# DeepLearningZ/chanamq

Hardware: AMD Instinct MI355X
Metric: msgs/sec (whole node) + p50 publish→deliver latency, 1 KB payload, 1/2/4/8 GPUs (higher is better)
Workload: dtype uint8 (AMQP wire bytes; no floating-point compute)

## Files before the change

### csrc/kernels/dataplane.hip

```cpp
#include "dp_state.h"
#include "dp_util.h"

DEV void apply_deltas(const DS& d, const u8* buf, u32 tid, u32 nt, DeltaRec* lrec) {
  const DeltaHead h = *(const DeltaHead*)buf;
  const DeltaRec* recs = (const DeltaRec*)(buf + sizeof(DeltaHead));
  const u32* dirty = (const u32*)(recs + h.nrec);
  const uint4* data = (const uint4*)((const u8*)dirty + ((4u * h.ndirty + 15u) & ~15u));
  for (u32 r = tid; r < h.nrec; r += nt) lrec[r] = recs[r];
  __syncthreads();
  for (u32 i = tid; i < h.nchunk; i += nt) {
    u32 lo = 0, hi = h.nrec;
    while (hi - lo > 1) {
      const u32 mid = (lo + hi) >> 1;
      if (lrec[mid].chunk0 <= i) lo = mid; else hi = mid;
    }
    const DeltaRec r = lrec[lo];
    const u32 off = (i - r.chunk0) * 16u;
    const u32 n = r.len - off < 16u ? r.len - off : 16u;
    const uint4 v = data[i];
    u8* dst = (u8*)(uintptr_t)(r.dst + off);
    const u32 w[4] = {v.x, v.y, v.z, v.w};
    if (((uintptr_t)dst & 3) == 0 && (n & 3) == 0) {
      for (u32 k = 0; k < n / 4; ++k) ((u32*)dst)[k] = w[k];
    } else {
// ... 77 lines not shown
    const u32 o = block_scan<1024>(v, lds, all);
    if (k < nseg) { d.seg_total[k] = cl + len; d.seg_start[k] = run + o; }
    run += all;
  }
}

#include "dp_frame_scan.h"

DEV void set_counts(const DS& d, u32 np, u32 na) {
  d.ctr->n_pubs = np < d.pub_max ? np : d.pub_max;
  d.ctr->n_acks = na < d.ack_max ? na : d.ack_max;
  d.tot[TS_RANGE_LO] = 0;
  d.tot[TS_RANGE_HI] = d.ctr->n_pubs;
  d.tot[TS_PAIR_BASE] = 0;
  d.tot[TS_PAIR_N] = 0;
  d.tot[TS_NIMPORT] = 0;
}

DEV bool skip_shortstr(const u8* p, u32& o, u32 end) {
  if (o + 1 > end) return false;
  o += 1 + p[o];
  return o <= end;
}

DEV u32 build_keyvec(const DS& d, const u8* key, u32 len, u32 pi) {
  Words kw = words_of(key, len);
  if (d.tb_max) {
    uint4* kv = (uint4*)(d.pub_keyvec + (u64)pi * TOPIC_K);
    u16* kwo = d.pub_kwoff + (u64)pi * TOPIC_WORDS;
    u32 off = 0;
    u32 wi = 0;
    if (kw.count) {
      while (wi < TOPIC_WORDS && off <= kw.eff) {
        u32 wl = word_len(key, off, kw.eff);
        u32 h = fnv1a32(key + off, wl);
        kwo[wi] = (u16)((off << 8) | (wl & 255));
        u32 pk[8];
#pragma unroll
        for (int g = 0; g < 8; ++g) {
          u32 v = 0;
#pragma unroll
          for (int bb = 0; bb < 4; ++bb) v |= (((h >> (g * 4 + bb)) & 1) ? 0x01u : 0xffu) << (8 * bb);
          pk[g] = v;
        }
        kv[wi * 2] = make_uint4(pk[0], pk[1], pk[2], pk[3]);
        kv[wi * 2 + 1] = make_uint4(pk[4], pk[5], pk[6], pk[7]);
        off += wl + 1;
        ++wi;
      }
    }
    for (; wi < TOPIC_WORDS; ++wi) {
      kv[wi * 2] = make_uint4(0, 0, 0, 0);
      kv[wi * 2 + 1] = make_uint4(0, 0, 0, 0);
    }
  }
  return kw.count;
}

struct Win32 { u32 w0, w1, w2, w3, w4, w5, w6, w7; };
DEV Win32 load_win(const u8* p) {
  const U4 a = *(const U4*)p, b = *(const U4*)(p + 16);
  return Win32{a.x, a.y, a.z, a.w, b.x, b.y, b.z, b.w};
}
DEV u32 win_word(const Win32& s, u32 k) {
  const u32 a0 = s.w0, a1 = s.w1, a2 = s.w2, a3 = s.w3, a4 = s.w4, a5 = s.w5, a6 = s.w6, a7 = s.w7;
  const u32 lo = k < 2 ? (k == 0 ? a0 : a1) : (k == 2 ? a2 : a3);
  const u32 hi = k < 6 ? (k == 4 ? a4 : a5) : (k == 6 ? a6 : a7);
  return k < 4 ? lo : hi;
}
DEV u32 win_byte(const Win32& s, u32 i) { return (win_word(s, i >> 2) >> (8 * (i & 3))) & 255u; }
DEV u32 win_get(const Win32& s, u32 i) { return win_byte(s, i); }
template <u32 S>
DEV u64 win_fnv64(const Win32& s, u32 n, u64 h) {
#pragma unroll
  for (u32 i = 0; i + S < 32; ++i) {
    if (i < n) {
      h ^= win_byte(s, i + S);
      h *= FNV64_PRIME;
    }
  }
  return h;
}

DEV u32 build_keyvec_win(const DS& d, const Win32& s, u32 n, u32 pi) {
  const u32 lenmask = n >= 32 ? ~0u : ((1u << n) - 1u);
  u32 dots = 0;
#pragma unroll
  for (u32 i = 0; i < 32; ++i) dots |= (win_byte(s, i) == '.' ? 1u : 0u) << i;
  dots &= lenmask;
  const u32 nd = ~dots & lenmask;
  const u32 eff = nd ? 32u - __clz(nd) : 0u;
  const u32 effmask = eff >= 32 ? ~0u : ((1u << eff) - 1u);
  const u32 de = dots & effmask;
  const u32 count = n == 0 ? 1u : (eff == 0 ? 0u : 1u + __popc(de));
  if (!d.tb_max) return count;
  u32 hw[TOPIC_WORDS];
#pragma unroll
  for (u32 k = 0; k < TOPIC_WORDS; ++k) hw[k] = 0x811c9dc5u;
  u32 h = 0x811c9dc5u, wi = 0;
#pragma unroll
  for (u32 i = 0; i < 32; ++i) {
    const u32 c = win_byte(s, i);
    const bool in = i < eff, dot = in && c == '.';
#pragma unroll
    for (u32 k = 0; k < TOPIC_WORDS; ++k) hw[k] = (dot && wi == k) ? h : hw[k];
    wi += dot ? 1u : 0u;
    h = dot ? 0x811c9dc5u : (in ? (h ^ c) * 0x01000193u : h);
  }
#pragma unroll
  for (u32 k = 0; k < TOPIC_WORDS; ++k) hw[k] = wi == k ? h : hw[k];
  const u32 nw = count < TOPIC_WORDS ? count : TOPIC_WORDS;
  uint4* kv = (uint4*)(d.pub_keyvec + (u64)pi * TOPIC_K);
  u16* kwo = d.pub_kwoff + (u64)pi * TOPIC_WORDS;
  u32 off = 0;
#pragma unroll
  for (u32 k = 0; k < TOPIC_WORDS; ++k) {
    if (k < nw) {
      const u32 rest = off >= 32 ? 0u : (de & ~((1u << off) - 1u));
      u32 e = rest ? (u32)(__ffs(rest) - 1) : eff;
      if (e > eff) e = eff;
      const u32 wl = e - off;
      kwo[k] = (u16)((off << 8) | (wl & 255));
      u32 pk[8];
#pragma unroll
      for (int g = 0; g < 8; ++g) {
        u32 v = 0;
#pragma unroll
        for (int bb = 0; bb < 4; ++bb) v |= (((hw[k] >> (g * 4 + bb)) & 1) ? 0x01u : 0xffu) << (8 * bb);
        pk[g] = v;
      }
      kv[k * 2] = make_uint4(pk[0], pk[1], pk[2], pk[3]);
      kv[k * 2 + 1] = make_uint4(pk[4], pk[5], pk[6], pk[7]);
      off = e + 1;
    } else {
      kv[k * 2] = make_uint4(0, 0, 0, 0);
      kv[k * 2 + 1] = make_uint4(0, 0, 0, 0);
    }
  }
  return count;
}

DEV void apply_ack(const DS& d, Ack a, u32 ai) {
  const u32 ch = a.chslot;
  if (ch == INVALID) { d.acks[ai] = a; return; }
  const u64 nt = d.ch_next_tag[ch];
  u64 tag = a.tag;
  if (tag == 0 && a.multiple) tag = nt - 1;
  a.tag = tag;
  d.acks[ai] = a;
  const bool requeue = (a.kind != CK_ACK) && a.requeue;
  if (a.multiple) {
    atomicMin(&d.ch_mlo[ch], ai);
    atomicMax(&d.ch_mhi[ch], ai);
  } else if (tag >= d.ch_uhead[ch] && tag < nt) {
    USlot& u = d.uwin[(u64)ch * (d.ucap_mask + 1) + ((tag - 1) & d.ucap_mask)];
    atomicCAS(&u.state, (u32)US_PENDING, requeue ? (u32)US_REQUEUE : (u32)US_ACKED);
  }
  if (atomicExch(&d.ch_dirty[ch], 1u) == 0) {
    u32 k = atomicAdd(d.n_dirty, 1u);
    d.dirty_list[k] = ch;
  }
  atomicAdd(&d.ctr->n_acked, 1u);
}

__global__ __launch_bounds__(256) void k_decode(DS d) {
  __shared__ u32 spref[DEC_SEG_LDS];
  __shared__ u32 sprefa[DEC_SEG_LDS];
  __shared__ u32 lds[256 / 64 + 1];
  const u32 nseg = d.in->nseg;
  const bool seg_order = nseg <= DEC_SEG_LDS;
  u32 n0 = d.ctr->n_cmds;
  n0 = n0 < d.cmd_max ? n0 : d.cmd_max;
  if (!d.rank_scan) {
    if (blockIdx.x != 0 && blockIdx.x * 256 >= n0) return;
    u32 run = 0, runa = 0;
    for (u32 b0 = 0; b0 < nseg; b0 += 256) {
      const u32 k = b0 + threadIdx.x;
      const u32 v = k < nseg ? d.seg_npub[k] : 0, va = k < nseg ? d.seg_nack[k] : 0;
      u32 all, alla;
      const u32 o = block_scan<256>(v, lds, all);
      const u32 oa = block_scan<256>(va, lds, alla);
      if (k < nseg) { spref[k] = run + o; sprefa[k] = runa + oa; }
      run += all;
      runa += alla;
    }
    if (blockIdx.x == 0 && threadIdx.x == 0) set_counts(d, run, runa);
    __syncthreads();
    if (blockIdx.x * 256 >= n0) return;
  } else {
    if (blockIdx.x == 0 && threadIdx.x == 0) set_counts(d, d.tot[TS_CMD_PUBS], d.tot[TS_CMD_ACKS]);
    if (blockIdx.x * 256 >= n0) return;
    if (seg_order) {
      u32 run = 0;
      for (u32 b0 = 0; b0 < nseg; b0 += 256) {
        const u32 k = b0 + threadIdx.x;
        const u32 v = k < nseg ? d.seg_npub[k] : 0;
        u32 all;
        const u32 o = block_scan<256>(v, lds, all);
        if (k < nseg) spref[k] = run + o;
        run += all;
      }
      __syncthreads();
    }
  }
  u32 i = blockIdx.x * blockDim.x + threadIdx.x;
  u32 n = d.ctr->n_cmds;
  if (n > d.cmd_max) n = d.cmd_max;
  if (i >= n) return;
  const Cmd c = d.cmds[i];
  const u8* w = d.work;
  if (c.kind == CK_PUBLISH) {
    u32 pi;
    if (!d.rank_scan) {
      pi = spref[c.seg] + c.pad[1];
    } else {
      pi = d.cmd_pub_rank[i];
      if (seg_order && c.seg < nseg && d.seg_cmd_base[c.seg] != INVALID)
        pi = spref[c.seg] + (pi - d.cmd_pub_rank[d.seg_cmd_base[c.seg]]);
    }
    if (pi >= d.pub_max) return;
    Pub pb;
    pb.conn = c.conn;
    pb.chslot = c.pad[0];
    pb.frag0 = c.frag0;
    pb.nfrag = c.nfrag;
    pb.body_size = c.body_size;
    pb.flags = 0;
    pb.expire_ms = 0;
    pb.ts_ms = 0;
    pb.nq = 0; pb.slot_bytes = 0; pb.msg = INVALID; pb.pad = 0; pb.xid = 0;
    u32 o = c.m_off + 6, end = c.m_off + c.m_len;
    const u32 o0 = o;
    const Win32 ma = load_win(w + o0);
    bool ok = o <= end;
    pb.ex_off = o + 1;
    const u32 b0 = ok && o < end ? win_byte(ma, 0) : 0u;
    pb.ex_len = b0;
    if (ok) { if (o + 1 > end) ok = false; else { o += 1 + b0; ok = o <= end; } }
    pb.rk_off = o + 1;
    const u32 b1 = ok && o < end ? (o - o0 < 32 ? win_get(ma, o - o0) : (u32)w[o]) : 0u;
    pb.rk_len = b1;
    if (ok) { if (o + 1 > end) ok = false; else { o += 1 + b1; ok = o <= end; } }
    const Win32 rkw = load_win(w + pb.rk_off);
    u32 bits = (ok && o < end) ? (o - pb.rk_off < 32 ? win_get(rkw, o - pb.rk_off) : (u32)w[o]) : 0u;
    if (bits & 1) pb.flags |= MF_MANDATORY;
    if (bits & 2) pb.flags |= MF_IMMEDIATE;
    i32 xs = -1;
    if (ok) {
      const u32 vh = d.conn_vhost[c.conn];
      u64 hk = pb.ex_len <= 31 ? win_fnv64<1>(ma, pb.ex_len, FNV64_BASIS ^ (u64(vh) * 0x9E3779B97F4A7C15ULL))
                               : exch_hash(vh, w + pb.ex_off, pb.ex_len);
      u32 mask = d.xhash_mask;
      for (u32 j = 0; j <= mask; ++j) {
        u32 slot = (u32)(hk + j) & mask;
        i32 v = d.x_hval[slot];
        if (v < 0) break;
        if (d.x_hkey[slot] == hk) { xs = v; break; }
      }
    }
    pb.exch = ok ? xs : -2;
    pb.keyhash = pb.rk_len <= 32 ? win_fnv64<0>(rkw, pb.rk_len, FNV64_BASIS) : fnv1a64_dev(w + pb.rk_off, pb.rk_len);
    u32 ho = c.h_off + 12, hend = c.h_off + c.h_len;
    pb.props_off = ho;
    pb.props_len = hend > ho ? hend - ho : 0;
    const Win32 pw = load_win(w + ho);
    auto pbyte = [&](u32 q) -> u32 { const u32 o = q - ho; return o < 32 ? win_byte(pw, o) : (u32)w[q]; };
    u32 fl = 0;
    u32 nfl = 0;
    u32 q = ho;
    while (q + 2 <= hend) {
      u32 fw = (pbyte(q) << 8) | pbyte(q + 1);
      q += 2;
      if (nfl == 0) fl = fw;
      ++nfl;
      if (!(fw & 1)) break;
    }
    bool pok = true;
    for (int bit = 15; bit >= 2 && pok; --bit) {
      if (!(fl & (1u << bit))) continue;
      switch (bit) {
        case 13: {
          if (q + 4 > hend) { pok = false; break; }
          u32 tl = (pbyte(q) << 24) | (pbyte(q + 1) << 16) | (pbyte(q + 2) << 8) | pbyte(q + 3);
          q += 4 + tl;
          pok = q <= hend;
          break;
        }
        case 12:
          if (q + 1 > hend) { pok = false; break; }
          if (pbyte(q) == 2) pb.flags |= MF_PERSIST;
          q += 1;
          break;
        case 11: q += 1; pok = q <= hend; break;
        case 8: {
          if (q + 1 > hend) { pok = false; break; }
          u32 sl = pbyte(q);
          if (q + 1 + sl > hend) { pok = false; break; }
          i64 v = 0;
          bool digits = sl > 0 && sl <= 18;
          for (u32 k = 0; k < sl && digits; ++k) {
            u32 ch = pbyte(q + 1 + k);
            if (ch < '0' || ch > '9') digits = false;
            else v = v * 10 + (ch - '0');
          }
          if (digits) pb.expire_ms = d.in->now_ms + v;
          q += 1 + sl;
          break;
        }
        case 6: {
          if (q + 8 > hend) { pok = false; break; }
          u64 ts = 0;
#pragma unroll
          for (u32 k = 0; k < 8; ++k) ts = (ts << 8) | pbyte(q + k);
          pb.ts_ms = (i64)ts * 1000;
          pb.flags |= MF_HAS_TS;
          q += 8;
          break;
        }
        default:
          if (q + 1 > hend) { pok = false; break; }
          q += 1 + pbyte(q);
          pok = q <= hend;
      }
    }
    pb.nwords = pb.rk_len <= 32 ? build_keyvec_win(d, rkw, pb.rk_len, pi) : build_keyvec(d, w + pb.rk_off, pb.rk_len, pi);
    if (c.nfrag == 1 && d.in->ingress_host && d.in->ref_back != 0xffffffffu && c.body_size >= d.in->ref_min &&
        c.seg < nseg) {
      const Frag fg = d.frags[c.frag0];
      const u32 w0 = d.seg_start[c.seg], cl = d.seg_total[c.seg] - d.segs[c.seg].len;
      const u64 ing_rel = (u64)d.in->ingress - (u64)d.work;
      if (fg.len == c.body_size && d.scan_inplace && (u64)d.in->ingress > (u64)d.work && fg.off >= ing_rel) {
        pb.flags |= MF_HREF;
        pb.pad = (u32)(fg.off - ing_rel);
      } else if (fg.len == c.body_size && fg.off >= w0 + cl && fg.off < w0 + d.seg_total[c.seg]) {
        pb.flags |= MF_HREF;
        pb.pad = (u32)(d.segs[c.seg].src + (fg.off - w0 - cl));
      }
    }
    d.pubs[pi] = pb;
  } else if (c.kind == CK_ACK || c.kind == CK_NACK || c.kind == CK_REJECT) {
    const u32 ai = d.rank_scan ? d.cmd_ack_rank[i] : sprefa[c.seg] + c.pad[2];
    if (ai >= d.ack_max) return;
    Ack a;
    a.chslot = c.pad[0];
    a.kind = c.kind;
    u32 o = c.m_off + 4;
    bool ok = c.m_len >= 13;
    a.tag = ok ? be64(w + o) : 0;
    u32 bits = ok ? w[o + 8] : 0;
    if (c.kind == CK_ACK) { a.multiple = bits & 1; a.requeue = 0; }
    else if (c.kind == CK_REJECT) { a.multiple = 0; a.requeue = bits & 1; }
    else { a.multiple = bits & 1; a.requeue = (bits >> 1) & 1; }
    d.acks[ai] = a;
  }
}

DEV void marks_range(const DS& d, u32 i0, u32 stride) {
  if (i0 == 0 && d.links)
    for (u32 r = 0; r < WORLD_MAX; ++r) d.lk_cnt[r] = 0;
  const u32 na = d.ctr->n_acks, np = d.ctr->n_pubs;
  const u32 n = na > np ? na : np;
  for (u32 i = i0; i < n; i += stride) {
    if (i < na) apply_ack(d, d.acks[i], i);
    if (i < np) {
      const u32 ch = d.pubs[i].chslot;
      if (ch != INVALID && d.ch_confirm[ch]) atomicAdd(&d.ch_pub_cnt[ch], 1u);
    }
  }
}

struct ScanArgs { const u32* in[4]; u32* out[4]; const u32* n; const u32* lo; u32 narr; u32 nmax; u32 tot_slot; u64 stride; };
#define SCAN_TILE 4096
template <int NA, int EPT>
DEV bool scan_tile(const ScanArgs& a, u32* tot, u64* status, u32* ctl, u32 smax) {
  constexpr u32 TILE = 1024 * EPT;
  __shared__ u32 s_tile, s_epoch;
  __shared__ u32 s_excl[NA];
  __shared__ u32 wsum[NA][1024 / 64 + 1];
  const u32 tid = threadIdx.x;
  if (tid == 0) {
    s_epoch = atomicAdd(&ctl[1], 0u);
    s_tile = atomicAdd(&ctl[0], 1u);
  }
  __syncthreads();
  const u32 tile = s_tile, epoch = s_epoch & 0x3fffffffu;
  const bool last_block = tile == gridDim.x - 1;
  u32 n = a.n ? *a.n : a.nmax;
  if (n > a.nmax) n = a.nmax;
  const u32 lo = a.lo ? *a.lo : 0u;
  n = n > lo ? n - lo : 0;
  const u32 base = tile * TILE;
  const bool data = base < n || tile == 0;
  if (data) {
    const u32 i = base + tid * EPT;
    u32 v[NA][EPT], off[NA], sm[NA];
#pragma clang loop unroll(full)
    for (int k = 0; k < NA; ++k) {
#pragma clang loop unroll(full)
      for (int e = 0; e < EPT; ++e) v[k][e] = 0;
      if ((u32)k >= a.narr) continue;
      const u32* in = (NA <= 4 ? a.in[k & 3] : a.in[k & 1] + (u64)(k >> 1) * a.stride) + lo;
      if (EPT == 4 && i + 3 < n && !(((uintptr_t)(in + i)) & 15)) {
        uint4 x = *(const uint4*)(in + i);
        v[k][0] = x.x; v[k][EPT > 1 ? 1 : 0] = x.y; v[k][EPT > 2 ? 2 : 0] = x.z; v[k][EPT > 3 ? 3 : 0] = x.w;
      } else {
#pragma clang loop unroll(full)
        for (int e = 0; e < EPT; ++e)
          if (i + e < n) v[k][e] = in[i + e];
      }
    }
    const u32 ln = tid & 63, w = tid >> 6;
    u32 x[NA];
#pragma clang loop unroll(full)
    for (int k = 0; k < NA; ++k) {
      u32 t = 0;
#pragma clang loop unroll(full)
      for (int e = 0; e < EPT; ++e) t += v[k][e];
      sm[k] = t;
      x[k] = t;
    }
#pragma clang loop unroll(full)
    for (int o = 1; o < 64; o <<= 1) {
#pragma clang loop unroll(full)
// ... 1124 lines not shown
  if (need <= cap) return;
  const u64 limit = d.q_max_cap[q] ? d.q_max_cap[q] : d.ring_pool;
  u64 want = cap;
  while (want < 2 * need && want * 2 <= limit) want *= 2;
  if (want <= cap) return;
  unsigned long long* top = (unsigned long long*)d.ring_top;
  u64 off = __hip_atomic_load(top, __ATOMIC_RELAXED, __HIP_MEMORY_SCOPE_AGENT);
  while (true) {
    if (off + want > d.ring_pool) return;
    u64 prev = atomicCAS(top, off, off + want);
    if (prev == off) break;
    off = prev;
  }
  RingMove mv;
  mv.q = q; mv.pad = 0;
  mv.old_off = d.q_ring_off[q]; mv.old_mask = mask;
  mv.new_off = off; mv.new_mask = want - 1;
  mv.head = head; mv.tail = tail;
  const u32 mi = atomicAdd(&d.tot[TS_NMOVE], 1u);
  d.moves[mi] = mv;
  d.q_ring_off[q] = off;
  d.q_ring_mask[q] = want - 1;
  const u32 gi = atomicAdd(&d.ctr->n_grow, 1u);
  if (gi < GROW_MAX) d.grow_h[gi] = mv;
  __threadfence();
}

__global__ __launch_bounds__(256) void k_ring_plan(DS d, u32 src) {
  __shared__ u32 s_last;
  const u32 n = d.tot[TS_PAIR_N];
  u32 nb = (n + 255) / 256;
  if (nb > gridDim.x) nb = gridDim.x;
  if (blockIdx.x >= nb) return;
  for (u32 i = blockIdx.x * 256 + threadIdx.x; i < n; i += gridDim.x * 256) ring_plan_one(d, src, i, n);
  __builtin_amdgcn_fence(__ATOMIC_RELEASE, "workgroup");
  __syncthreads();
  if (threadIdx.x == 0) s_last = atomicAdd(&d.tot[TS_RP_TICKET], 1u) == nb - 1;
  __syncthreads();
  if (!s_last) return;
  __builtin_amdgcn_fence(__ATOMIC_ACQUIRE, "agent");
  if (threadIdx.x == 0) d.tot[TS_RP_TICKET] = 0;
  copy_moved_rings(d, d.tot[TS_NMOVE], threadIdx.x, 256);
}

__global__ void k_enqueue(DS d, u32 src) {
  const u32 n = d.tot[TS_PAIR_N];
  const u32 stride = gridDim.x * blockDim.x;
  for (u32 b = blockIdx.x * blockDim.x; b < n; b += stride) {
    const u32 i = b + threadIdx.x;
    PersistRec pr;
    pr.msg = INVALID;
    u32 drop = i < n ? enqueue_one(d, src, i, n, &pr) : INVALID;
    enqueue_done(d, drop, pr);
  }
}

DEV void plan_rings_block(const DS& d, const u32* hscan, u32 n, u32 D, u32 tid, u32 nt) {
  const u32 rb = d.rank_bits;
  for (u32 q = tid; q < d.q_max && (q << rb) < D; q += nt) {
    const u32 first = __hip_atomic_load(&hscan[q << rb], __ATOMIC_RELAXED, __HIP_MEMORY_SCOPE_AGENT);
    const u32 nx = ((q + 1) << rb) < D
                       ? __hip_atomic_load(&hscan[(q + 1) << rb], __ATOMIC_RELAXED, __HIP_MEMORY_SCOPE_AGENT)
                       : n;
    if (nx > first) plan_queue(d, q, nx - first);
  }
  __syncthreads();
  const u32 nm = __hip_atomic_load(&d.tot[TS_NMOVE], __ATOMIC_RELAXED, __HIP_MEMORY_SCOPE_AGENT);
  if (!nm) return;
  __builtin_amdgcn_fence(__ATOMIC_ACQUIRE, "agent");
  copy_moved_rings(d, nm, tid, nt);
}

template <int DB>
__global__ __launch_bounds__(RsNt<DB>::v) void k_rs_hist_plan(DS d, const u32* keys, const u32* np, u32* hist,
                                                             u32* hscan, u32* ticket, u32 ntiles) {
  const u32 n = *np;
  if (n == 0) return;
  if (!rs_hist_tiles<DB>(keys, n, 0u, hist, hscan, ticket, ntiles)) return;
  __builtin_amdgcn_fence(__ATOMIC_RELEASE, "workgroup");
  __syncthreads();
  plan_rings_block(d, hscan, n, 1u << DB, threadIdx.x, RsNt<DB>::v);
}

template <int DB>
__global__ __launch_bounds__(256) void k_rs_scatter_enq(DS d, const u32* kin, const u32* vin, const u32* np,
                                                       const u32* hscan) {
  constexpr u32 D = 1u << DB, CH = SORT_TILE / 256;
  __shared__ u32 wc[4][D];
  const u32 tid = threadIdx.x, w = tid >> 6, lane = tid & 63;
  const u32 n = *np, rb = d.rank_bits;
  const u64 lt = lanemask_lt();
  for (u32 t = blockIdx.x; t * SORT_TILE < n; t += gridDim.x) {
    const u32 base = t * SORT_TILE;
    __syncthreads();
    for (u32 i = tid; i < 4 * D; i += 256) ((u32*)wc)[i] = 0;
    __syncthreads();
    const u32 wbase = base + w * (SORT_TILE / 4);
    u32 key[CH], val[CH];
    u64 pe[CH];
#pragma unroll
    for (u32 c = 0; c < CH; ++c) {
      const u32 i = wbase + c * 64 + lane;
      key[c] = i < n ? kin[i] : 0u;
      val[c] = i < n ? vin[i] : 0u;
    }
#pragma unroll
    for (u32 c = 0; c < CH; ++c) {
      const bool valid = wbase + c * 64 + lane < n;
      const u32 dg = key[c] & (D - 1);
      const u64 peers = pe[c] = digit_peers<DB>(dg, valid);
      if (valid && ((peers & lt) == 0)) wc[w][dg] += __popcll(peers);
      __builtin_amdgcn_wave_barrier();
    }
    __syncthreads();
    for (u32 dg = tid; dg < D; dg += 256) {
      u32 run = hscan[t * D + dg];
      for (u32 ww = 0; ww < 4; ++ww) { const u32 x = wc[ww][dg]; wc[ww][dg] = run; run += x; }
    }
    __syncthreads();
    u32 pos[CH];
#pragma unroll
    for (u32 c = 0; c < CH; ++c) {
      const bool valid = wbase + c * 64 + lane < n;
      const u32 dg = key[c] & (D - 1);
      const u32 basepos = ((volatile u32*)wc[w])[dg];
      pos[c] = basepos + __popcll(pe[c] & lt);
      __builtin_amdgcn_wave_barrier();
      if (valid && ((pe[c] & lt) == 0)) ((volatile u32*)wc[w])[dg] = basepos + __popcll(pe[c]);
      __builtin_amdgcn_wave_barrier();
    }
    EnqLoad el[CH];
    u32 first[CH], nx[CH];
#pragma unroll
    for (u32 c = 0; c < CH; ++c) {
      const bool valid = wbase + c * 64 + lane < n;
      const u32 q = key[c] >> rb;
      first[c] = valid ? hscan[q << rb] : 0u;
      nx[c] = valid ? (((q + 1) << rb) < D ? hscan[(q + 1) << rb] : n) : 0u;
      el[c] = valid ? enq_load(d, q, val[c]) : EnqLoad{};
    }
#pragma unroll
    for (u32 c = 0; c < CH; ++c) {
      const bool valid = wbase + c * 64 + lane < n;
      PersistRec pr;
      pr.msg = INVALID;
      u32 drop = INVALID;
      if (valid) drop = enq_store(d, el[c], key[c] >> rb, pos[c] - first[c], pos[c] + 1 == nx[c], &pr);
      enqueue_done(d, drop, pr);
    }
  }
}

DEV bool wants_record(const DS& d, u32 msg, u32 q, bool valid) {
  return d.persist && valid && msg != INVALID && d.q_durable[q] && (d.msgs[msg].flags & MF_PERSIST);
}
DEV void consumed_rec_at(const DS& d, u32 msg, u32 q, u64 qpos, u32 kind, u32 k) {
  ConsumedRec r;
  r.msg_id = (i64)d.msgs[msg].msg_id;
  r.qpos = qpos;
  r.q = q;
  r.kind = kind;
  r.pad[0] = r.pad[1] = 0;
  d.crec[k] = r;
}
DEV void link_consumed(const DS& d, u32 msg, u32 q, u32 kind, bool valid) {
  if (d.links && valid && msg != INVALID && kind <= 2u) {
    const u32 ow = d.q_link_owner[q];
    if (ow) {
      const u32 k = atomicAdd(&d.lk_cnt[ow - 1], 1u);
      if (k < d.lk_cap) {
        AckRec a;
        a.tq = q;
        a.pad = 0;
        a.xid = d.msgs[msg].msg_id;
        d.lk_send[(u64)(ow - 1) * d.lk_cap + k] = a;
      }
    }
  }
}
DEV void wave_consumed(const DS& d, u32 msg, u32 q, u64 qpos, u32 kind, bool valid) {
  link_consumed(d, msg, q, kind, valid);
  if (!d.persist) return;
  bool want = wants_record(d, msg, q, valid);
  u32 k = wave_reserve(&d.ctr->n_consumed, want);
  if (want && k < d.persist_max) consumed_rec_at(d, msg, q, qpos, kind, k);
}


#define MS_MAX 256
struct MsLds {
  u64 up[MS_MAX + 1];
  u32 rq[MS_MAX + 1];
  u32 wc[4];
  u32 rc[4];
  u32 rbase;
  u32 n, nb;
  unsigned long long ovf_a, ovf_r;
};
DEV void chan_advance_one(const DS& d, u32 ch, u32 tid, u32 lane, u32 w, u32* s_first, u32* s_done, MsLds& ms);
__global__ __launch_bounds__(256) void k_chan_advance(DS d) {
  __shared__ u32 s_first[4];
  __shared__ u32 s_done[4];
  __shared__ MsLds ms;
  const u32 tid = threadIdx.x, lane = lane_id(), w = tid >> 6;
  const u32 nd = *d.n_dirty;
  for (u32 wv = blockIdx.x; wv < nd; wv += gridDim.x) chan_advance_one(d, d.dirty_list[wv], tid, lane, w, s_first,
                                                                        s_done, ms);
}

DEV void collect_settles(const DS& d, u32 ch, u32 tid, u32 lane, u32 w, MsLds& ms) {
  const u32 lo = d.ch_mlo[ch], hi = d.ch_mhi[ch];
  if (tid == 0) { ms.n = 0; ms.nb = 0; ms.ovf_a = 0; ms.ovf_r = 0; }
  __syncthreads();
  if (lo == INVALID) return;
  for (u32 base = lo; base <= hi; base += 256) {
    const u32 i = base + tid;
    bool take = false;
    Ack a;
    a.tag = 0; a.kind = 0; a.requeue = 0;
    if (i <= hi) {
      a = d.acks[i];
      take = a.chslot == ch && a.multiple;
    }
    const bool rq = (a.kind != CK_ACK) && a.requeue;
    const u64 m = __ballot(take);
    if (lane == 0) ms.wc[w] = (u32)__popcll(m);
    __syncthreads();
    u32 pos = ms.n + (u32)__popcll(m & lanemask_lt());
    for (u32 k = 0; k < w; ++k) pos += ms.wc[k];
    if (take) {
      if (pos < MS_MAX) { ms.up[pos] = a.tag; ms.rq[pos] = rq; }
      else atomicMax(rq ? &ms.ovf_r : &ms.ovf_a, (unsigned long long)a.tag);
    }
    __syncthreads();
    if (tid == 0) ms.n += ms.wc[0] + ms.wc[1] + ms.wc[2] + ms.wc[3];
    __syncthreads();
  }
  if (tid == 0) {
    const u32 n = ms.n < MS_MAX ? ms.n : MS_MAX;
    u64 top = 0;
    u32 nb = 0;
    for (u32 k = 0; k < n; ++k)
      if (ms.up[k] > top) { ms.up[nb] = ms.up[k]; ms.rq[nb] = ms.rq[k]; ++nb; top = ms.up[k]; }
    const u64 oa = ms.ovf_a, orq = ms.ovf_r;
    const u64 om = oa > orq ? oa : orq;
    if (om > top) { ms.up[nb] = om; ms.rq[nb] = orq > oa; ++nb; }
    ms.nb = nb;
    d.ch_mlo[ch] = INVALID;
    d.ch_mhi[ch] = 0;
  }
  __syncthreads();
}

DEV u32 ca_reserve(const DS& d, u32 n) {
  const u32 lim = d.persist_max - d.deliv_max - (d.persist_max >> 2) - 64u;
  u32 cur = *(volatile u32*)&d.ctr->n_consumed;
  while (true) {
    if (cur + n > lim) return INVALID;
    const u32 prev = atomicCAS(&d.ctr->n_consumed, cur, cur + n);
    if (prev == cur) return cur;
    cur = prev;
  }
}

DEV void chan_advance_one(const DS& d, u32 ch, u32 tid, u32 lane, u32 w, u32* s_first, u32* s_done, MsLds& ms) {
  collect_settles(d, ch, tid, lane, w, ms);
  const u32 nb = ms.nb;
  const u64 head = d.ch_uhead[ch], nt = d.ch_next_tag[ch];
  const u64 aup = d.ch_ack_upto[ch], rup = d.ch_req_upto[ch];
  USlot* win = d.uwin + (u64)ch * (d.ucap_mask + 1);
  bool contiguous = true;
  bool deferred = false;
  u64 newhead = head;
  u32 manual_done = 0;
  for (u64 t0 = head; t0 < nt; t0 += 256) {
    const u64 t = t0 + tid;
    const bool valid = t < nt;
    u32 st = US_FREE;
    USlot u;
    u.state = US_FREE; u.msg = INVALID; u.q = 0; u.cons = 0; u.qpos = 0; u.expire_ms = 0;
    if (valid) {
      u = win[(t - 1) & d.ucap_mask];
      st = u.state;
      if (st == US_PENDING) {
        if (t <= aup) st = US_ACKED;
        else if (t <= rup) st = US_REQUEUE;
        else
          for (u32 k = 0; k < nb; ++k)
            if (t <= ms.up[k]) { st = ms.rq[k] ? US_REQUEUE : US_ACKED; break; }
      }
    }
// ... 1656 lines not shown
```

### csrc/kernels/engine.hip

```cpp
#include <pybind11/pybind11.h>
#include <pybind11/numpy.h>
#include <pybind11/stl.h>

#include <chrono>
#include <algorithm>
#include <functional>
#include <map>
#include <memory>
#include <mutex>
#include <condition_variable>
#include <thread>
#include <type_traits>
#include <stdexcept>
#include <string>
#include <vector>

#include <hsa/amd_hsa_signal.h>
#include <hsa/hsa.h>
#include <hsa/hsa_ext_amd.h>
#include <rocprofiler-sdk-roctx/roctx.h>

#include "dataplane.hip"
#include "delta_stage.h"
#include "xchg_host.h"
// ... 2247 lines not shown
    a.dl_state = [](void* e, int which) -> u64 { return ((Engine*)e)->dl_state(which); };
    a.unpaused = [](void* e, int p, const u32** out) -> u32 {
      Engine* en = (Engine*)e;
      if (p < 0 || p >= en->npar_) return 0;
      *out = en->par_[p].stage_unp;
      return en->par_[p].nunp;
    };
    a.set_egress_ref = [](void* e, int back, u32 min_bytes) -> int {
      return ((Engine*)e)->guard([&] { ((Engine*)e)->set_egress_ref(back, min_bytes); return 0; });
    };
    return (u64)&api_;
  }

  template <class F>
  int guard(F&& f) {
    try {
      HIPCHECK(hipSetDevice(device_));
      return f();
    } catch (std::exception& ex) {
      err_ = ex.what();
      return -1;
    }
  }

 private:
  static ScanArgs scan_args(std::initializer_list<std::pair<const u32*, u32*>> arrs, const u32* n, u32 nmax,
                            u32 slot, const u32* lo) {
    if (arrs.size() > 4) throw std::runtime_error("launch_scan: at most 4 arrays");
    ScanArgs a{};
    a.lo = lo;
    u32 k = 0;
    for (auto& p : arrs) { a.in[k] = p.first; a.out[k] = p.second; ++k; }
    a.narr = k;
    a.n = n;
    a.nmax = nmax;
    a.tot_slot = slot;
    return a;
  }
  void launch_scan(hipStream_t s, const DS& d, std::initializer_list<std::pair<const u32*, u32*>> arrs, const u32* n,
                   u32 nmax, u32 slot, const u32* lo = nullptr, bool ingest = false) {
    const ScanArgs a = scan_args(arrs, n, nmax, slot, lo);
    u32 nb = ceil_div(nmax ? nmax : 1, SCAN_TILE);
    hipLaunchKernelGGL((k_scan<4, 4>), dim3(nb), dim3(1024), 0, s, a, d.tot, ingest ? scan_status_ing_ : scan_status_,
                       ingest ? scan_ctl_ing_ : scan_ctl_, scan_smax_);
  }
  template <class F>
  static void with_key_bits(u32 bits, F&& f) {
    if (bits <= 8) f(std::integral_constant<u32, 8>{});
    else if (bits == 9) f(std::integral_constant<u32, 9>{});
    else if (bits == 10) f(std::integral_constant<u32, 10>{});
    else f(std::integral_constant<u32, 11>{});
  }
  u32 radix_sort(hipStream_t s, const DS& d, u32** keys, u32** vals, const u32* n, u32 nmax, u32 bits) {
    const u32 ntiles = ceil_div(nmax, SORT_TILE);
    const u32 digit = bits > 8 && bits <= 11 ? bits : 8;
    u32 src = 0;
    for (u32 shift = 0; shift < bits; shift += digit) {
      with_key_bits(digit, [&](auto b) {
        constexpr u32 B = decltype(b)::value;
        hipLaunchKernelGGL(k_rs_hist<B>, capped(ntiles, 256), dim3(RsNt<B>::v), 0, s, keys[src], n, shift, d_.hist,
                           d_.hist_scan, &d.tot[TS_RS_TICKET], ntiles);
        hipLaunchKernelGGL(k_rs_scatter<B>, capped(ntiles, 256), dim3(256), 0, s, keys[src], vals[src], keys[src ^ 1],
                           vals[src ^ 1], n, shift, d_.hist_scan, ntiles);
      });
      src ^= 1;
    }
    return src;
  }

  static dim3 blocks(u64 n, u32 per) { return dim3(n ? ceil_div(n, per) : 1); }
  static dim3 wave_blocks(u64 n) { u64 b = n ? ceil_div(n, 4) : 1; return dim3(b > 8192 ? 8192 : (u32)b); }
  static dim3 capped(u64 b, u32 cap) { return dim3(b == 0 ? 1u : (b > cap ? cap : (u32)b)); }

  void launch_ingest(hipStream_t s, const DS& d) {
    Range rg("chanamq.K1-K4.ingest");
    hipLaunchKernelGGL(k_stage, dim3(1), dim3(1024), 0, s, d);
    const dim3 fs_grid = capped(d.seg_max, n_cu_);
    const bool fold = h2d_hsa_ && fs_grid.x >= 16;
    if (h2d_hsa_ && !fold) hipLaunchKernelGGL(k_h2d_wait, dim3(16), dim3(64), 0, s, d);
    hipLaunchKernelGGL(k_frame_scan, fs_grid, dim3(FS_NT), 0, s, d, fold ? 1u : 0u);
    if (d.rank_scan)
      launch_scan(s, d, {{d.cmd_is_pub, d.cmd_pub_rank}, {d.cmd_is_ack, d.cmd_ack_rank}}, &d.ctr->n_cmds,
                  d.cmd_max, TS_CMD_PUBS, nullptr, true);
    hipLaunchKernelGGL(k_decode, blocks(d.cmd_max, 256), dim3(256), 0, s, d);
  }

  void launch_route(hipStream_t s, const DS& d, u32 nmax, bool imports = false) {
    Range rg("chanamq.K6-K13.route_store");
    const u64 ngroups = ceil_div(nmax ? nmax : 1, 16);
    if (imports) hipLaunchKernelGGL(k_import_route, capped(ngroups, n_cu_), dim3(1024), 0, s, d);
    else hipLaunchKernelGGL(k_route, capped(ngroups, 2 * n_cu_), dim3(1024), 0, s, d);
    const ScanArgs a = scan_args({{d.pub_nq, d.pub_pair_off}, {d.pub_slot, d.pub_slot_off},
                                  {d.pub_routed, d.pub_routed_rank}, {d.pub_ret_sz, d.pub_ret_off}},
                                 &d.tot[TS_RANGE_HI], d.pub_cap, TS_ROUTE, &d.tot[TS_RANGE_LO]);
    hipLaunchKernelGGL(k_scan_route, dim3(ceil_div(d.pub_cap ? d.pub_cap : 1, SCAN_TILE)), dim3(1024), 0, s, a, d.tot,
                       scan_status_, scan_ctl_, scan_smax_, d);
    hipLaunchKernelGGL(k_route_store, wave_blocks(nmax), dim3(256), 0, s, d, imports ? 0u : 1u);
  }

  void launch_pack(hipStream_t s, const DS& d) {
    Range rg("chanamq.X1.pack");
    hipLaunchKernelGGL(k_pack_scan, blocks(d.pub_max, PK_TILE), dim3(1024), 0, s, d, d.pk_agg, &d.tot[TS_PK_TICKET]);
    hipLaunchKernelGGL(k_pack, wave_blocks(d.pub_max), dim3(256), 0, s, d);
  }

  void launch_tail(hipStream_t s, const DS& d, bool dispatch = true) {
    Range rg("chanamq.K7-K11.tail");
    u32 nch = d.c_max * d.chpc;
    const u32 pbits = d.q_bits + d.rank_bits;
    if (pbits <= 11) {
      const u32 nt = ceil_div(d.pair_max, SORT_TILE);
      const u32* n = &d.tot[TS_PAIR_N];
      u32* tk = &d.tot[TS_RS_TICKET];
      with_key_bits(pbits, [&](auto b) {
        constexpr u32 B = decltype(b)::value;
        hipLaunchKernelGGL(k_rs_hist_plan<B>, capped(nt, 256), dim3(RsNt<B>::v), 0, s, d, d.pair_k[0], n, d_.hist, d_.hist_scan, tk, nt);
        hipLaunchKernelGGL(k_rs_scatter_enq<B>, capped(nt, 256), dim3(256), 0, s, d, d.pair_k[0], d.pair_v[0], n, d_.hist_scan);
      });
    } else {
      u32* pk[2] = {d.pair_k[0], d.pair_k[1]};
      u32* pv[2] = {d.pair_v[0], d.pair_v[1]};
      const u32 psrc = radix_sort(s, d, pk, pv, &d.tot[TS_PAIR_N], d.pair_max, pbits);
      hipLaunchKernelGGL(k_qfirst, blocks(d.pair_max, 256), dim3(256), 0, s, d, psrc);
      hipLaunchKernelGGL(k_ring_plan, capped(ceil_div(d.pair_max, 256), 1024), dim3(256), 0, s, d, psrc);
      hipLaunchKernelGGL(k_enqueue, capped(ceil_div(d.pair_max, 256), 1024), dim3(256), 0, s, d, psrc);
    }
    const u32 fin = d.persist ? 0u : 1u;
    if (!dispatch) {
      const u64 pn = d.deliv_max > d.c_max ? d.deliv_max : d.c_max;
      hipLaunchKernelGGL(k_post, blocks(pn, 256), dim3(256), 0, s, d, fin);
      if (!fin) hipLaunchKernelGGL(k_host_out, dim3(64), dim3(256), 0, s, d);
      return;
    }
    hipLaunchKernelGGL(k_chan_advance, capped(nch, 1024), dim3(256), 0, s, d);
    hipLaunchKernelGGL(k_dequeue, dim3(d.q_max), dim3(256), 0, s, d);
    hipLaunchKernelGGL(k_dv_write, blocks(d.deliv_max, 256), dim3(256), 0, s, d);
    if (d.c_max <= CONN_LAYOUT_MAX) {
      hipLaunchKernelGGL(k_conn_layout, dim3(1), dim3(1024), 0, s, d);
    } else {
      launch_scan(s, d, {{d.dv_size, d.dv_off}}, &d.ctr->n_deliv, d.deliv_max, TS_DELIV_BYTES);
      hipLaunchKernelGGL(k_conn_sizes, blocks(d.c_max, 256), dim3(256), 0, s, d);
      launch_scan(s, d, {{d.conn_total, d.conn_base}}, nullptr, d.c_max, TS_CONN_BYTES);
      hipLaunchKernelGGL(k_conn_out, blocks(d.c_max, 256), dim3(256), 0, s, d);
    }
    if (d.links) hipLaunchKernelGGL(k_link_bases, dim3(1), dim3(64), 0, s, d);
    {
      const u32 n_rc = RC_RET_BLOCKS + ceil_div(d.c_max, 256);
      hipLaunchKernelGGL(k_render, dim3(n_rc + wave_blocks(d.deliv_max).x), dim3(256), 0, s, d, n_rc);
    }
    u64 pn = d.deliv_max > d.c_max ? d.deliv_max : d.c_max;
    hipLaunchKernelGGL(k_post, blocks(pn, 256), dim3(256), 0, s, d, fin);
    if (d.persist) {
      hipLaunchKernelGGL(k_persist_size, blocks(d.persist_max, 256), dim3(256), 0, s, d);
      launch_scan(s, d, {{d.ps_size, d.ps_off}}, &d.ctr->n_persist, d.persist_max, TS_PERSIST);
      hipLaunchKernelGGL(k_persist_pack, wave_blocks(d.persist_max), dim3(256), 0, s, d);
      hipLaunchKernelGGL(k_host_out, dim3(64), dim3(256), 0, s, d);
    }
  }

  void launch_main(hipStream_t s, const DS& d) {
    launch_ingest(s, d);
    launch_route(s, d, d.pub_max);
    if (d.world > 1) launch_pack(s, d);
    else launch_tail(s, d);
  }

  void launch_rest(hipStream_t s, const DS& d) {
    launch_route(s, d, d.pub_max);
    launch_tail(s, d);
  }
  void capture(hipStream_t st, hipGraphExec_t* ge, const std::function<void()>& f) {
    hipGraph_t g;
    std::lock_guard<std::mutex> cg(cap_mu_);
    HIPCHECK(hipStreamBeginCapture(st, hipStreamCaptureModeThreadLocal));
    f();
    HIPCHECK(hipStreamEndCapture(st, &g));
    HIPCHECK(hipGraphInstantiate(ge, g, nullptr, nullptr, 0));
    HIPCHECK(hipGraphDestroy(g));
  }

  void launch_phase_b(hipStream_t s, const DS& d, bool dispatch = true) {
    Range rg("chanamq.X1.import");
    launch_route(s, d, d.import_max, true);
    launch_tail(s, d, dispatch);
  }
};

static py::array alloc_pinned(size_t bytes) {
  void* p = nullptr;
  HIPCHECK(hipHostMalloc(&p, bytes, hipHostMallocPortable));
  return py::array(py::dtype("uint8"), {(py::ssize_t)bytes}, {(py::ssize_t)1}, p,
                   py::capsule(p, [](void* q) { (void)hipHostFree(q); }));
}

static u64 create_stream(int device) {
  HIPCHECK(hipSetDevice(device));
  hipStream_t st;
  HIPCHECK(hipStreamCreateWithFlags(&st, hipStreamNonBlocking));
  return (u64)st;
}

static int device_count() {
  int n = 0;
  if (hipGetDeviceCount(&n) != hipSuccess) return 0;
  return n;
}

PYBIND11_MODULE(_dataplane, m) {
  m.doc() = "MI355X (gfx950) AMQP data-plane kernels + native step runtime";
  m.def("alloc_pinned", &alloc_pinned, "page-locked host buffer (numpy uint8)");
  m.def("roctx_push", [](const std::string& n) { roctxRangePushA(n.c_str()); });
  m.def("roctx_pop", []() { roctxRangePop(); });
  m.def("roctx_mark", [](const std::string& n) { roctxMarkA(n.c_str()); });
  m.def("device_count", &device_count);
  m.def("create_stream", &create_stream, py::arg("device") = 0);
  m.attr("CAND_MAX") = CAND_MAX;
  m.attr("TOPIC_K") = TOPIC_K;
// ... 87 lines not shown
```

Measured before the change: 49.60 million.

## Split routing-key hashing across lanes and fold channel advance into scatter kernel

Decoding now gives each publish TOPIC_WORDS threads, with each lane hashing one topic word of a short routing key and writing its own key-vector slot. The per-bit byte expansion is replaced by a multiply-and-mask trick. For small sort keys, the channel-advance work runs in extra blocks appended to the radix scatter/enqueue launch, reusing that kernel's LDS and removing a separate launch. This trades more threads per command and grid-stride looping for less serial per-thread work. Sort blocks and channel-advance blocks now share one grid.

Result: faster. 50.27 million, median of 4 (+1.4%).

```diff
diff --git a/csrc/kernels/dataplane.hip b/csrc/kernels/dataplane.hip
--- a/csrc/kernels/dataplane.hip
+++ b/csrc/kernels/dataplane.hip
@@ -183,7 +183,7 @@
   return h;
 }
 
-DEV u32 build_keyvec_win(const DS& d, const Win32& s, u32 n, u32 pi) {
+DEV u32 build_keyvec_lane(const DS& d, const Win32& s, u32 n, u32 pi, u32 k) {
   const u32 lenmask = n >= 32 ? ~0u : ((1u << n) - 1u);
   u32 dots = 0;
 #pragma unroll
@@ -195,49 +195,31 @@
   const u32 de = dots & effmask;
   const u32 count = n == 0 ? 1u : (eff == 0 ? 0u : 1u + __popc(de));
   if (!d.tb_max) return count;
-  u32 hw[TOPIC_WORDS];
-#pragma unroll
-  for (u32 k = 0; k < TOPIC_WORDS; ++k) hw[k] = 0x811c9dc5u;
-  u32 h = 0x811c9dc5u, wi = 0;
+  const u32 nw = count < TOPIC_WORDS ? count : TOPIC_WORDS;
+  uint4* kv = (uint4*)(d.pub_keyvec + (u64)pi * TOPIC_K) + k * 2;
+  if (k >= nw) {
+    kv[0] = make_uint4(0, 0, 0, 0);
+    kv[1] = make_uint4(0, 0, 0, 0);
+    return count;
+  }
+  u32 rest = de, off = 0;
+#pragma unroll
+  for (u32 j = 0; j + 1 < TOPIC_WORDS; ++j)
+    if (j < k) { off = (u32)__ffs(rest); rest &= rest - 1u; }
+  u32 e = rest ? (u32)(__ffs(rest) - 1) : eff;
+  if (e > eff) e = eff;
+  u32 h = 0x811c9dc5u;
 #pragma unroll
   for (u32 i = 0; i < 32; ++i) {
     const u32 c = win_byte(s, i);
-    const bool in = i < eff, dot = in && c == '.';
-#pragma unroll
-    for (u32 k = 0; k < TOPIC_WORDS; ++k) hw[k] = (dot && wi == k) ? h : hw[k];
-    wi += dot ? 1u : 0u;
-    h = dot ? 0x811c9dc5u : (in ? (h ^ c) * 0x01000193u : h);
-  }
-#pragma unroll
-  for (u32 k = 0; k < TOPIC_WORDS; ++k) hw[k] = wi == k ? h : hw[k];
-  const u32 nw = count < TOPIC_WORDS ? count : TOPIC_WORDS;
-  uint4* kv = (uint4*)(d.pub_keyvec + (u64)pi * TOPIC_K);
-  u16* kwo = d.pub_kwoff + (u64)pi * TOPIC_WORDS;
-  u32 off = 0;
-#pragma unroll
-  for (u32 k = 0; k < TOPIC_WORDS; ++k) {
-    if (k < nw) {
-      const u32 rest = off >= 32 ? 0u : (de & ~((1u << off) - 1u));
-      u32 e = rest ? (u32)(__ffs(rest) - 1) : eff;
-      if (e > eff) e = eff;
-      const u32 wl = e - off;
-      kwo[k] = (u16)((off << 8) | (wl & 255));
-      u32 pk[8];
-#pragma unroll
-      for (int g = 0; g < 8; ++g) {
-        u32 v = 0;
-#pragma unroll
-        for (int bb = 0; bb < 4; ++bb) v |= (((hw[k] >> (g * 4 + bb)) & 1) ? 0x01u : 0xffu) << (8 * bb);
-        pk[g] = v;
-      }
-      kv[k * 2] = make_uint4(pk[0], pk[1], pk[2], pk[3]);
-      kv[k * 2 + 1] = make_uint4(pk[4], pk[5], pk[6], pk[7]);
-      off = e + 1;
-    } else {
-      kv[k * 2] = make_uint4(0, 0, 0, 0);
-      kv[k * 2 + 1] = make_uint4(0, 0, 0, 0);
-    }
-  }
+    h = (i >= off && i < e) ? (h ^ c) * 0x01000193u : h;
+  }
+  d.pub_kwoff[(u64)pi * TOPIC_WORDS + k] = (u16)((off << 8) | ((e - off) & 255));
+  u32 pk[8];
+#pragma unroll
+  for (int g = 0; g < 8; ++g) pk[g] = 0xffffffffu - ((((h >> (g * 4)) & 15u) * 0x00204081u) & 0x01010101u) * 0xfeu;
+  kv[0] = make_uint4(pk[0], pk[1], pk[2], pk[3]);
+  kv[1] = make_uint4(pk[4], pk[5], pk[6], pk[7]);
   return count;
 }
 
@@ -264,6 +246,8 @@
   atomicAdd(&d.ctr->n_acked, 1u);
 }
 
+#define DEC_CPB (256 / TOPIC_WORDS)
+DEV void decode_cmd(const DS& d, u32 i, u32 sub, const u32* spref, const u32* sprefa, bool seg_order, u32 nseg);
 __global__ __launch_bounds__(256) void k_decode(DS d) {
   __shared__ u32 spref[DEC_SEG_LDS];
   __shared__ u32 sprefa[DEC_SEG_LDS];
@@ -273,7 +257,7 @@
   u32 n0 = d.ctr->n_cmds;
   n0 = n0 < d.cmd_max ? n0 : d.cmd_max;
   if (!d.rank_scan) {
-    if (blockIdx.x != 0 && blockIdx.x * 256 >= n0) return;
+    if (blockIdx.x != 0 && blockIdx.x * DEC_CPB >= n0) return;
     u32 run = 0, runa = 0;
     for (u32 b0 = 0; b0 < nseg; b0 += 256) {
       const u32 k = b0 + threadIdx.x;
@@ -287,10 +271,10 @@
     }
     if (blockIdx.x == 0 && threadIdx.x == 0) set_counts(d, run, runa);
     __syncthreads();
-    if (blockIdx.x * 256 >= n0) return;
+    if (blockIdx.x * DEC_CPB >= n0) return;
   } else {
     if (blockIdx.x == 0 && threadIdx.x == 0) set_counts(d, d.tot[TS_CMD_PUBS], d.tot[TS_CMD_ACKS]);
-    if (blockIdx.x * 256 >= n0) return;
+    if (blockIdx.x * DEC_CPB >= n0) return;
     if (seg_order) {
       u32 run = 0;
       for (u32 b0 = 0; b0 < nseg; b0 += 256) {
@@ -304,10 +288,12 @@
       __syncthreads();
     }
   }
-  u32 i = blockIdx.x * blockDim.x + threadIdx.x;
-  u32 n = d.ctr->n_cmds;
-  if (n > d.cmd_max) n = d.cmd_max;
-  if (i >= n) return;
+  const u32 sub = threadIdx.x % TOPIC_WORDS;
+  for (u32 i = blockIdx.x * DEC_CPB + threadIdx.x / TOPIC_WORDS; i < n0; i += gridDim.x * DEC_CPB)
+    decode_cmd(d, i, sub, spref, sprefa, seg_order, nseg);
+}
+
+DEV void decode_cmd(const DS& d, u32 i, u32 sub, const u32* spref, const u32* sprefa, bool seg_order, u32 nseg) {
   const Cmd c = d.cmds[i];
   const u8* w = d.work;
   if (c.kind == CK_PUBLISH) {
@@ -424,7 +410,9 @@
           pok = q <= hend;
       }
     }
-    pb.nwords = pb.rk_len <= 32 ? build_keyvec_win(d, rkw, pb.rk_len, pi) : build_keyvec(d, w + pb.rk_off, pb.rk_len, pi);
+    if (pb.rk_len <= 32) pb.nwords = build_keyvec_lane(d, rkw, pb.rk_len, pi, sub);
+    else if (sub == 0) pb.nwords = build_keyvec(d, w + pb.rk_off, pb.rk_len, pi);
+    if (sub != 0) return;
     if (c.nfrag == 1 && d.in->ingress_host && d.in->ref_back != 0xffffffffu && c.body_size >= d.in->ref_min &&
         c.seg < nseg) {
       const Frag fg = d.frags[c.frag0];
@@ -439,7 +427,7 @@
       }
     }
     d.pubs[pi] = pb;
-  } else if (c.kind == CK_ACK || c.kind == CK_NACK || c.kind == CK_REJECT) {
+  } else if (sub == 0 && (c.kind == CK_ACK || c.kind == CK_NACK || c.kind == CK_REJECT)) {
     const u32 ai = d.rank_scan ? d.cmd_ack_rank[i] : sprefa[c.seg] + c.pad[2];
     if (ai >= d.ack_max) return;
     Ack a;
@@ -1730,15 +1718,40 @@
   plan_rings_block(d, hscan, n, 1u << DB, threadIdx.x, RsNt<DB>::v);
 }
 
+#define MS_MAX 256
+struct MsLds {
+  u64 up[MS_MAX + 1];
+  u32 rq[MS_MAX + 1];
+  u32 wc[4];
+  u32 rc[4];
+  u32 rbase;
+  u32 n, nb;
+  unsigned long long ovf_a, ovf_r;
+};
+struct CaLds { MsLds ms; u32 s_first[4]; u32 s_done[4]; };
+DEV void chan_advance_one(const DS& d, u32 ch, u32 tid, u32 lane, u32 w, u32* s_first, u32* s_done, MsLds& ms);
+DEV void chan_advance_blocks(const DS& d, u32 blk, u32 nblk, CaLds& l) {
+  const u32 tid = threadIdx.x, lane = lane_id(), w = tid >> 6;
+  const u32 nd = *d.n_dirty;
+  for (u32 wv = blk; wv < nd; wv += nblk) chan_advance_one(d, d.dirty_list[wv], tid, lane, w, l.s_first, l.s_done, l.ms);
+}
+__global__ __launch_bounds__(256) void k_chan_advance(DS d) {
+  __shared__ CaLds l;
+  chan_advance_blocks(d, blockIdx.x, gridDim.x, l);
+}
+
 template <int DB>
 __global__ __launch_bounds__(256) void k_rs_scatter_enq(DS d, const u32* kin, const u32* vin, const u32* np,
-                                                       const u32* hscan) {
+                                                       const u32* hscan, u32 n_ca) {
   constexpr u32 D = 1u << DB, CH = SORT_TILE / 256;
-  __shared__ u32 wc[4][D];
+  __shared__ __attribute__((aligned(8))) u32 wc[4][D];
+  static_assert(sizeof(CaLds) <= sizeof(wc), "the window-advance blocks use the digit counts' LDS");
+  const u32 nsort = gridDim.x - n_ca;
+  if (blockIdx.x >= nsort) { chan_advance_blocks(d, blockIdx.x - nsort, n_ca, *(CaLds*)&wc[0][0]); return; }
   const u32 tid = threadIdx.x, w = tid >> 6, lane = tid & 63;
   const u32 n = *np, rb = d.rank_bits;
   const u64 lt = lanemask_lt();
-  for (u32 t = blockIdx.x; t * SORT_TILE < n; t += gridDim.x) {
+  for (u32 t = blockIdx.x; t * SORT_TILE < n; t += nsort) {
     const u32 base = t * SORT_TILE;
     __syncthreads();
     for (u32 i = tid; i < 4 * D; i += 256) ((u32*)wc)[i] = 0;
@@ -1834,27 +1847,6 @@
   if (want && k < d.persist_max) consumed_rec_at(d, msg, q, qpos, kind, k);
 }
 
-
-#define MS_MAX 256
-struct MsLds {
-  u64 up[MS_MAX + 1];
-  u32 rq[MS_MAX + 1];
-  u32 wc[4];
-  u32 rc[4];
-  u32 rbase;
-  u32 n, nb;
-  unsigned long long ovf_a, ovf_r;
-};
-DEV void chan_advance_one(const DS& d, u32 ch, u32 tid, u32 lane, u32 w, u32* s_first, u32* s_done, MsLds& ms);
-__global__ __launch_bounds__(256) void k_chan_advance(DS d) {
-  __shared__ u32 s_first[4];
-  __shared__ u32 s_done[4];
-  __shared__ MsLds ms;
-  const u32 tid = threadIdx.x, lane = lane_id(), w = tid >> 6;
-  const u32 nd = *d.n_dirty;
-  for (u32 wv = blockIdx.x; wv < nd; wv += gridDim.x) chan_advance_one(d, d.dirty_list[wv], tid, lane, w, s_first,
-                                                                        s_done, ms);
-}
 
 DEV void collect_settles(const DS& d, u32 ch, u32 tid, u32 lane, u32 w, MsLds& ms) {
   const u32 lo = d.ch_mlo[ch], hi = d.ch_mhi[ch];
diff --git a/csrc/kernels/engine.hip b/csrc/kernels/engine.hip
--- a/csrc/kernels/engine.hip
+++ b/csrc/kernels/engine.hip
@@ -2353,7 +2353,7 @@
     if (d.rank_scan)
       launch_scan(s, d, {{d.cmd_is_pub, d.cmd_pub_rank}, {d.cmd_is_ack, d.cmd_ack_rank}}, &d.ctr->n_cmds,
                   d.cmd_max, TS_CMD_PUBS, nullptr, true);
-    hipLaunchKernelGGL(k_decode, blocks(d.cmd_max, 256), dim3(256), 0, s, d);
+    hipLaunchKernelGGL(k_decode, capped(ceil_div(d.cmd_max, DEC_CPB), 2 * n_cu_), dim3(256), 0, s, d);
   }
 
   void launch_route(hipStream_t s, const DS& d, u32 nmax, bool imports = false) {
@@ -2383,10 +2383,12 @@
       const u32 nt = ceil_div(d.pair_max, SORT_TILE);
       const u32* n = &d.tot[TS_PAIR_N];
       u32* tk = &d.tot[TS_RS_TICKET];
+      const u32 n_ca = dispatch ? capped(nch, 1024).x : 0u;
       with_key_bits(pbits, [&](auto b) {
         constexpr u32 B = decltype(b)::value;
         hipLaunchKernelGGL(k_rs_hist_plan<B>, capped(nt, 256), dim3(RsNt<B>::v), 0, s, d, d.pair_k[0], n, d_.hist, d_.hist_scan, tk, nt);
-        hipLaunchKernelGGL(k_rs_scatter_enq<B>, capped(nt, 256), dim3(256), 0, s, d, d.pair_k[0], d.pair_v[0], n, d_.hist_scan);
+        hipLaunchKernelGGL(k_rs_scatter_enq<B>, dim3(capped(nt, 256).x + n_ca), dim3(256), 0, s, d, d.pair_k[0], d.pair_v[0], n,
+                           d_.hist_scan, n_ca);
       });
     } else {
       u32* pk[2] = {d.pair_k[0], d.pair_k[1]};
@@ -2403,7 +2405,7 @@
       if (!fin) hipLaunchKernelGGL(k_host_out, dim3(64), dim3(256), 0, s, d);
       return;
     }
-    hipLaunchKernelGGL(k_chan_advance, capped(nch, 1024), dim3(256), 0, s, d);
+    if (pbits > 11) hipLaunchKernelGGL(k_chan_advance, capped(nch, 1024), dim3(256), 0, s, d);
     hipLaunchKernelGGL(k_dequeue, dim3(d.q_max), dim3(256), 0, s, d);
     hipLaunchKernelGGL(k_dv_write, blocks(d.deliv_max, 256), dim3(256), 0, s, d);
     if (d.c_max <= CONN_LAYOUT_MAX) {
diff --git a/profiles/short_chain/ab_summary.py b/profiles/short_chain/ab_summary.py
--- /dev/null
+++ b/profiles/short_chain/ab_summary.py
@@ -0,0 +1,27 @@
+#!/usr/bin/env python3
+import json
+import re
+import statistics
+import sys
+
+rows = [json.loads(line) for line in open(sys.argv[1]) if line.strip()]
+runs = [dict(kind=r["kind"], build=r["build"], msgs_per_s=r["result"]["value"], us_per_step=r["result"]["ms_per_step"] * 1e3,
+             p50_latency_ms=r["result"]["p50_latency_ms"], p99_latency_ms=r["result"]["p99_latency_ms"]) for r in rows]
+plain = {b: [r for r in runs if r["kind"] == "plain" and r["build"] == b] for b in ("parent", "change")}
+summ = {b: dict(runs=len(v), median_msgs_per_s=statistics.median(r["msgs_per_s"] for r in v),
+                lowest_msgs_per_s=min(r["msgs_per_s"] for r in v),
+                median_p50_ms=statistics.median(r["p50_latency_ms"] for r in v),
+                lowest_p50_ms=min(r["p50_latency_ms"] for r in v)) for b, v in plain.items()}
+gate = dict(p50_ok=summ["change"]["median_p50_ms"] < summ["parent"]["lowest_p50_ms"],
+            throughput_ok=summ["change"]["median_msgs_per_s"] >= summ["parent"]["lowest_msgs_per_s"])
+doc = dict(commands={"plain": "python bench.py --gpus 1 --steps 50 --warmup 10", "steps200": "... --steps 200 --warmup 10",
+                     "chunk32k": "... --steps 50 --warmup 10 --chunk 32768"},
+           runs=runs, summary=summ, gate=gate)
+if len(sys.argv) > 3:
+    probe = open(sys.argv[3]).read()
+    doc["copy_probe_us"] = {k: float(m.group(1)) for k, pat in (("engine_0", r"^hsa +engine 0,.*?: ([\d.]+) us"),
+                                                                 ("two_engines", r"^split engines.*?: ([\d.]+) us"))
+                            for m in [re.search(pat, probe, re.M)] if m}
+with open(sys.argv[2], "w") as f:
+    json.dump(doc, f, indent=1)
+print(json.dumps(dict(summary=summ, gate=gate, probe=doc.get("copy_probe_us")), indent=1))
```
